# titisda/graph-python

Hardware: AMD Instinct MI355X
Metric: GTEPS (masked mxv/vxm level-BFS, R-MAT s22) (higher is better)
Workload: dtype bool; 1 GPU; level-BFS q<!v.S,replace> = q any.pair A (GxB_ANY_PAIR_BOOL; GrB_vxm, GrB_mxv on A^T shards for N>1), R-MAT scale 22, edge factor 16, 16 roots; n=4194304, nnz=65243197, parallelism=single GPU

## Files before the change

### graph-python_amd/csrc/gb_internal.h

```cpp
#pragma once
#include <atomic>
#include <utility>
#include <hip/hip_runtime.h>

#include <cstdint>
#include <cstring>
#include <stdexcept>
#include <string>
#include <vector>

#include "../../include/gbamd_codes.h"
#include "gb_state.h"
#include "../../include/graphblas_amd.h"

#define GB_MAGIC 0x6d614d424731ULL
#define GB_FREED 0x646565724642ULL

struct GB_Type_opaque {
    uint64_t magic;
    int code;
    size_t size;
    const char *name;
};
struct GB_BinaryOp_opaque {
// ... 1 lines not shown
    int opcode;
    GrB_Type xtype, ytype, ztype;
    const char *name;
};
struct GB_UnaryOp_opaque {
    uint64_t magic;
    int opcode;
    GrB_Type xtype, ztype;
    const char *name;
};
struct GB_IndexUnaryOp_opaque {
    uint64_t magic;
    int opcode;
    GrB_Type xtype, ytype;
    const char *name;
};
struct GB_Monoid_opaque {
    uint64_t magic;
    int mcode;
    GrB_Type type;
    GrB_BinaryOp op;
    const char *name;
};
struct GB_Semiring_opaque {
    uint64_t magic;
    GrB_Monoid add;
    GrB_BinaryOp mul;
    const char *name;
    bool user;
};
struct GB_Descriptor_opaque {
    uint64_t magic;
    int outp, mask, inp0, inp1;
    bool builtin;
    const char *name;
};

struct GB_builtin_entry {
    const char *name;
    int kind;
    void *obj;
};
extern const GB_builtin_entry GB_builtin_registry[];

enum { GB_KIND_MATRIX = 0, GB_KIND_VECTOR = 1, GB_KIND_SCALAR = 2 };

struct gb_orient_cache {
    int32_t *hub_tab = nullptr;
    int64_t hub_n = 0, hub_H = 0;
    uint64_t *rows_ne = nullptr;
    uint32_t *ne_rank = nullptr;
    int32_t *phead = nullptr;
    uint32_t *pdeg = nullptr;
    int64_t maxdeg = -1;
    int32_t *long_tab = nullptr;
    int64_t long_n = 0;
    int32_t *hot_ci = nullptr;
    int32_t *hot_cols = nullptr;
    int64_t hot_n = 0;
    void *nar_vx = nullptr;
    int nar_k = 0;
    bool nar_done = false;
};
void gb_orient_cache_drop(gb_orient_cache &c);

struct GB_Matrix_opaque {
    uint64_t magic;
    int kind;
    GrB_Type type;
    int64_t nrows, ncols;
    bool iso;
    int64_t nvals;
    int64_t *rowptr;
    int32_t *colidx;
    void *vals;
    bool t_valid;
    int64_t *t_rowptr;
    int32_t *t_colidx;
    void *t_vals;
    int64_t *t_perm;
    gb_orient_cache oc[2];
    uint64_t *bits;
    void *dense;
    int64_t *d_nvals;
    bool nvals_valid;
    struct gb_host_slot *pub;
    uint64_t pub_seq, pub_epoch;
    bool hint_valid;
    const void *hint_key;
    std::string err;
    uint64_t *cw;
    void *cw_vals;
    int64_t *cw_stat;
    GrB_Info invalid = GrB_SUCCESS;
};
typedef GB_Matrix_opaque GB_Obj;

inline GB_Obj *OBJ(const void *p) { return (GB_Obj *)p; }

struct gb_exception {
    GrB_Info info;
    std::string msg;
};
[[noreturn]] void gb_throw(GrB_Info info, const std::string &msg);
#define GB_REQUIRE(cond, info, msg) \
    do {                            \
// ... 104 lines not shown
void *gb_malloc(size_t bytes);
void gb_free(void *p);
template <class T>
T *gb_malloc_n(size_t n) {
    return (T *)gb_malloc(n * sizeof(T));
}
void gb_memset(void *p, int v, size_t bytes);
void gb_copy_d2d(void *dst, const void *src, size_t bytes);
void gb_copy_h2d(void *dst, const void *src, size_t bytes);
void gb_copy_d2h(void *dst, const void *src, size_t bytes);

struct gb_scratch {
    void *ptrs[32];
    int n = 0;
    template <class T>
    T *get(size_t count) {
        T *p = gb_malloc_n<T>(count ? count : 1);
        ptrs[n++] = p;
        return p;
    }
    ~gb_scratch() {
        for (int i = 0; i < n; i++) gb_free(ptrs[i]);
    }
};

GB_Obj *gb_obj_check(const void *p, bool allow_null = false);
GB_Obj *gb_obj_check_raw(const void *p, bool allow_null = false);
void gb_cw_to_csr(GB_Obj *A);
void gb_cw_release(GB_Obj *A);
void gb_cw_materialize(GB_Obj *A);
GB_Obj *gb_new_object(int kind, GrB_Type type, int64_t nrows, int64_t ncols);
extern "C" void gb_vec_recount(GB_Obj *v);
void gb_obj_free_storage(GB_Obj *A);
void gb_drop_transpose(GB_Obj *A);
int64_t gb_nvals(GB_Obj *A);
inline int64_t gb_words(int64_t n) { return (n + 63) >> 6; }
inline bool gb_is_bitmap(const GB_Obj *A) { return A->kind != GB_KIND_MATRIX; }

void gb_cast_array(void *dst, int dst_code, const void *src, int src_code, int64_t n);

struct gb_csr_view {
    int64_t nrows = 0, ncols = 0, nvals = 0;
    const int64_t *rowptr = nullptr;
    const int32_t *colidx = nullptr;
    const void *vals = nullptr;
    bool iso = false;
    int tcode = 0;
    const int32_t *hubs = nullptr;
    int64_t nhubs = 0, hub_H = 0;
    const uint64_t *nonempty = nullptr;
    const uint32_t *ne_rank = nullptr;
    const int32_t *phead = nullptr;
    const uint32_t *pdeg = nullptr;
    int64_t maxdeg = -1;
    const int32_t *lchunks = nullptr;
    int64_t nlchunks = -1;
    const void *nvx = nullptr;
    int nvk = 0;
    const int32_t *hcolidx = nullptr;
    const int32_t *hcols = nullptr;
    int64_t nhot = 0;
    gb_scratch own;
};
void gb_get_csr(gb_csr_view &v, GB_Obj *A);
void gb_view_hubs(gb_csr_view &v, GB_Obj *A, int orient, int64_t H);
void gb_view_nonempty(gb_csr_view &v, GB_Obj *A, int orient);
void gb_view_pullfirst(gb_csr_view &v, GB_Obj *A, int orient, const int64_t *other_rowptr, int64_t other_n);
void gb_view_long_rows(gb_csr_view &v, GB_Obj *A, int orient);
void gb_view_narrow(gb_csr_view &v, GB_Obj *A, int orient);
void gb_view_hot(gb_csr_view &v, GB_Obj *A, int orient);
void gb_get_csc(gb_csr_view &v, GB_Obj *A);
const int64_t *gb_csc_perm(GB_Obj *A);
const void *gb_view_vals_as(gb_csr_view &v, int code, gb_scratch &s);

struct gb_bitmap_view {
    int64_t n = 0;
    const uint64_t *bits = nullptr;
    const void *vals = nullptr;
    bool iso = false;
    int tcode = 0;
    const int64_t *count = nullptr;
    const long long *mf_hint = nullptr;
    const void *hint_key = nullptr;
    bool full = false;
    int64_t h_nvals = -1;
    gb_scratch own;
};
void gb_get_bitmap(gb_bitmap_view &v, GB_Obj *A);
const void *gb_bitmap_vals_as(gb_bitmap_view &v, int code, gb_scratch &s);

void gb_install_csr(GB_Obj *C, int64_t nrows, int64_t ncols, int64_t nvals, int64_t *rowptr,
                    int32_t *colidx, void *vals, bool iso);
void gb_install_bitmap(GB_Obj *C, int64_t n, uint64_t *bits, void *dense, bool iso,
                       int64_t *d_nvals );

void gb_bitmap_count(const uint64_t *bits, int64_t n, int64_t *d_count);
void gb_bitmap_to_csr(const uint64_t *bits, const void *dense, bool iso, int64_t n, size_t tsize,
                      int64_t **rowptr, int32_t **colidx, void **vals, int64_t *nvals);
void gb_csr_col_to_bitmap(const gb_csr_view &v, size_t tsize, uint64_t **bits, void **dense,
                          int64_t **d_nvals);

void gb_build(GB_Obj *C, const GrB_Index *I, const GrB_Index *J, const void *X, int xcode, bool x_iso,
              int64_t n, GrB_BinaryOp dup);
void gb_extract_tuples(GB_Obj *A, GrB_Index *I, GrB_Index *J, void *X, int xcode, GrB_Index *nvals);

void *gb_expand_iso(const void *one_value, size_t tsize, int64_t n);
// ... 163 lines not shown
```

### graph-python_amd/csrc/gb_mxv.hip

```cpp
#include "gb_dispatch.cuh"
#include "gb_internal.h"

#define SPMV_TILE 256

template <class SR, class X, class Z, bool FLIP>
__global__ __launch_bounds__(SPMV_BLOCK) void k_spmv_pull(
    SR sr, int64_t nrows, const int64_t *__restrict__ rowptr, const int32_t *__restrict__ colidx,
    const X *__restrict__ avals, bool a_iso, const uint64_t *__restrict__ ubits,
    const X *__restrict__ uvals, bool u_iso, const uint64_t *__restrict__ mbits, bool mcomp, int lg,
    uint64_t *__restrict__ tbits, Z *__restrict__ tvals, unsigned long long *__restrict__ tcount,
    unsigned long long *__restrict__ gst) {
    __shared__ unsigned long long words[SPMV_TILE / 64];
    const int G = 1 << lg;
    const int gid = threadIdx.x >> lg;
    const int gl = threadIdx.x & (G - 1);
    const int ngroups = SPMV_BLOCK >> lg;
    const int lane = threadIdx.x & 63;
    const unsigned long long gmask = (G == 64) ? ~0ULL : (((1ULL << G) - 1) << (lane & ~(G - 1)));
    const int64_t nwords = (nrows + 63) >> 6;
    const bool rv = SR::reads_values && avals && uvals;
    X a0 = X(), u0 = X();
    if (rv) {
        if (a_iso) a0 = avals[0];
        if (u_iso) u0 = uvals[0];
// ... 511 lines not shown
    const int64_t nw = (n + 63) >> 6;
    for (int64_t w = (blockIdx.x * (int64_t)blockDim.x + threadIdx.x) >> 6; w < nw;
         w += ((int64_t)gridDim.x * blockDim.x) >> 6) {
        const int64_t r = (w << 6) + lane;
        const unsigned long long b = __ballot(r < n && rowptr[r + 1] > rowptr[r]);
        if (lane == 0) {
            ne[w] = b;
            pc[w] = __popcll(b);
        }
    }
}

__global__ void k_narrow_u32(const int64_t *__restrict__ in, uint32_t *__restrict__ out, int64_t n) {
    GB_GRID_LOOP(i, n)
        out[i] = (uint32_t)in[i];
}

void gb_view_nonempty(gb_csr_view &v, GB_Obj *A, int orient) {
    if (A->kind != GB_KIND_MATRIX) return;
    gb_orient_cache &c = A->oc[orient];
    if (!c.rows_ne) {
        const int64_t nw = gb_words(v.nrows);
        c.rows_ne = gb_malloc_n<uint64_t>(nw);
        c.ne_rank = gb_malloc_n<uint32_t>(nw + 1);
        if (nw == 0) {
            gb_memset(c.ne_rank, 0, sizeof(uint32_t));
        } else {
            gb_scratch s;
            int32_t *pc = s.get<int32_t>(nw);
            int64_t *pre = s.get<int64_t>(nw + 1);
            const unsigned g = (unsigned)std::max<int64_t>(1, std::min<int64_t>((nw + 3) / 4, 8192));
            hipLaunchKernelGGL(k_rows_nonempty, dim3(g), dim3(256), 0, gb_stream(), v.rowptr, v.nrows, c.rows_ne, pc);
            GB_LAUNCH_CHECK();
            gb_exclusive_scan_i32(pc, 0, pre, nw);
            hipLaunchKernelGGL(k_narrow_u32, dim3(gb_grid(nw + 1, 256, 4096)), dim3(256), 0, gb_stream(), pre,
                               c.ne_rank, nw + 1);
            GB_LAUNCH_CHECK();
        }
    }
    v.nonempty = c.rows_ne;
    v.ne_rank = c.ne_rank;
}

__device__ __forceinline__ void pf_better(int64_t &bd, int32_t &bi, int64_t d, int32_t i) {
    if (i >= 0 && (d > bd || (d == bd && (bi < 0 || i < bi)))) {
        bd = d;
        bi = i;
    }
}
__global__ __launch_bounds__(256) void k_pull_head(int64_t n, const int64_t *__restrict__ rp,
                                                   const int32_t *__restrict__ ci,
                                                   const int64_t *__restrict__ orp, int64_t on,
                                                   const uint64_t *__restrict__ ne, const uint32_t *__restrict__ rank,
                                                   int4 *__restrict__ head, uint32_t *__restrict__ pdeg) {
    const int lane = threadIdx.x & 63;
    const int64_t nwaves = ((int64_t)gridDim.x * blockDim.x) >> 6;
    for (int64_t j = (blockIdx.x * (int64_t)blockDim.x + threadIdx.x) >> 6; j < n; j += nwaves) {
        const int64_t e0 = rp[j], e1 = rp[j + 1], d = e1 - e0;
        if (d <= 0) continue;
        const int64_t slot = (int64_t)rank[j >> 6] + __popcll(ne[j >> 6] & ((1ULL << (j & 63)) - 1));
        int32_t pick[4] = {-1, -1, -1, -1};
        const int rounds = d <= 4 ? (int)d : 3;
        for (int r = 0; r < rounds; r++) {
            int64_t bd = -1;
            int32_t bi = -1;
            for (int64_t e = e0 + lane; e < e1; e += 64) {
                const int32_t i = ci[e];
                bool taken = false;
                for (int q = 0; q < r; q++) taken = taken || pick[q] == i;
                if (!taken) pf_better(bd, bi, orp[i + 1] - orp[i], i);
            }
            for (int off = 32; off > 0; off >>= 1) {
                const int64_t od = __shfl_xor(bd, off, 64);
                const int32_t oi = __shfl_xor(bi, off, 64);
                pf_better(bd, bi, od, oi);
            }
            pick[r] = bi;
        }
        if (d > 4) pick[3] = -2;
        if (lane == 0) {
            head[slot] = make_int4(pick[0], pick[1], pick[2], pick[3]);
            if (pdeg) {
                const int64_t od = j < on ? orp[j + 1] - orp[j] : 0;
                pdeg[slot] = (uint32_t)(od < 0xFFFFFFFFLL ? od : 0xFFFFFFFFLL);
            }
        }
    }
}

void gb_view_pullfirst(gb_csr_view &v, GB_Obj *A, int orient, const int64_t *other_rowptr, int64_t other_n) {
    if (A->kind != GB_KIND_MATRIX || v.nrows == 0) return;
    gb_orient_cache &c = A->oc[orient];
    if (!c.rows_ne || !c.ne_rank || v.nonempty != c.rows_ne || v.ne_rank != c.ne_rank) return;
    if (!c.phead) {
        uint32_t ne_count = 0;
        gb_copy_d2h(&ne_count, c.ne_rank + gb_words(v.nrows), sizeof(ne_count));
        const int64_t nrec = std::max<int64_t>(1, (int64_t)ne_count);
        c.phead = gb_malloc_n<int32_t>(4 * nrec);
        c.pdeg = gb_malloc_n<uint32_t>(nrec);
        const unsigned g = (unsigned)std::max<int64_t>(1, std::min<int64_t>((v.nrows + 3) / 4, 65535));
        hipLaunchKernelGGL(k_pull_head, dim3(g), dim3(256), 0, gb_stream(), v.nrows, v.rowptr, v.colidx,
                           other_rowptr, other_n, c.rows_ne, c.ne_rank, reinterpret_cast<int4 *>(c.phead), c.pdeg);
        GB_LAUNCH_CHECK();
    }
    v.phead = c.phead;
    v.pdeg = c.pdeg;
}

static bool idempotent_monoid(int m) {
    return m == GBAMD_MON_ANY || m == GBAMD_MON_MIN || m == GBAMD_MON_MAX || m == GBAMD_MON_LOR ||
           m == GBAMD_MON_LAND || m == GBAMD_MON_BOR || m == GBAMD_MON_BAND;
}

bool gb_spmv_result_iso(GrB_Semiring sr, bool a_iso, bool u_iso, bool flip) {
    gb_sr_info info = gb_sr_describe(sr);
    bool reads_a = info.reads_values, reads_u = info.reads_values;
    if (info.mul == GBAMD_OP_FIRST) (flip ? reads_a : reads_u) = false;
    if (info.mul == GBAMD_OP_SECOND) (flip ? reads_u : reads_a) = false;
    if (info.mul == GBAMD_OP_PAIR) return idempotent_monoid(info.mon);
    return !info.positional && idempotent_monoid(info.mon) && (!reads_a || a_iso) && (!reads_u || u_iso);
}

template <class F>
static void gb_with_flip(bool flip, F &&f) {
    if (flip) f(std::true_type{});
    else f(std::false_type{});
}

void gb_spmv(gb_vec_result &T, const gb_csr_view &A, const gb_csr_view *Apush, gb_bitmap_view &u,
             const gb_vmask &mask, GrB_Semiring sr, bool flip, const gb_asg *asg) {
    gb_sr_info info = gb_sr_describe(sr);
    gb_scratch s;
    gb_csr_view &Av = const_cast<gb_csr_view &>(A);
    const void *av = info.reads_values ? gb_view_vals_as(Av, info.xcode, s) : nullptr;
    const void *uv = info.reads_values ? gb_bitmap_vals_as(u, info.xcode, s) : nullptr;
    const bool iso = gb_spmv_result_iso(sr, A.iso, u.iso, flip);

    const int64_t n = A.nrows;
    const size_t zs = gb_type_size(info.zcode);
    T.n = n;
    T.tcode = info.zcode;
    T.iso = iso;
    T.bits = gb_malloc_n<uint64_t>(gb_words(n));
    T.dense = gb_malloc((iso ? 1 : n) * zs);
    T.d_nvals = gb_malloc_n<int64_t>(2 + GB_HINT_PARTS);
    if (n == 0) {
        gb_memset(T.d_nvals, 0, sizeof(int64_t));
        return;
    }

    if (iso) {
        gb_spmv_iso(T, A, Apush, u, mask, sr, flip, asg, av, uv);
        return;
    }
    const int64_t nw = gb_words(n);
    unsigned long long *gst = gb_device_state();

    gb_dispatch_sr(info, [&](auto srf, auto x, auto z) {
        using SRT = decltype(srf);
// ... 54 lines not shown
```

### graph-python_amd/csrc/gb_object.hip

```cpp
#include <algorithm>
#include <vector>

#include <mutex>

#include "gb_dispatch.cuh"
#include "gb_internal.h"

#define GB_BLOCK 256
#define OBJ_GRID_CAP 8192

GB_Obj *gb_obj_check(const void *p, bool allow_null) {
    GB_Obj *A = gb_obj_check_raw(p, allow_null);
    if (A && A->cw) gb_cw_to_csr(A);
    return A;
}

GB_Obj *gb_obj_check_raw(const void *p, bool allow_null) {
    if (!p) {
        if (allow_null) return nullptr;
        gb_throw(GrB_NULL_POINTER, "required object is NULL");
    }
    GB_Obj *A = OBJ(p);
    if (A->magic == GB_FREED) gb_throw(GrB_INVALID_OBJECT, "object has been freed");
    if (A->magic != GB_MAGIC) gb_throw(GrB_UNINITIALIZED_OBJECT, "object is not initialized");
// ... 27 lines not shown
    GB_REQUIRE(type && type->magic == GB_MAGIC, GrB_UNINITIALIZED_OBJECT, "invalid type");
    GB_REQUIRE(nrows >= 0 && ncols >= 0, GrB_INVALID_VALUE, "negative dimension");
    GB_REQUIRE(nrows <= (int64_t)GrB_INDEX_MAX && ncols <= (int64_t)GrB_INDEX_MAX, GrB_INVALID_VALUE,
               "dimension too large");
    if (kind == GB_KIND_MATRIX) {
        GB_REQUIRE(ncols < (1LL << 31), GrB_OUT_OF_MEMORY,
                   "matrix with >= 2^31 columns exceeds the device index width");
    }
    GB_Obj *A = new GB_Obj();
    A->magic = GB_MAGIC;
    A->kind = kind;
    A->type = type;
    A->nrows = nrows;
    A->ncols = ncols;
    return A;
}

GB_Obj *gb_new_object(int kind, GrB_Type type, int64_t nrows, int64_t ncols) {
    GB_Obj *A = gb_new_object_bare(kind, type, nrows, ncols);
    try {
        alloc_empty_storage(A);
    } catch (...) {
        gb_free(A->rowptr);
        gb_free(A->bits);
        gb_free(A->d_nvals);
        A->magic = GB_FREED;
        delete A;
        throw;
    }
    return A;
}

void gb_drop_transpose(GB_Obj *A) {
    if (A->t_valid) {
        gb_free(A->t_rowptr);
        gb_free(A->t_colidx);
        gb_free(A->t_vals);
        gb_free(A->t_perm);
    }
    A->t_perm = nullptr;
    A->t_rowptr = nullptr;
    A->t_colidx = nullptr;
    A->t_vals = nullptr;
    A->t_valid = false;
    for (gb_orient_cache &c : A->oc) gb_orient_cache_drop(c);
}

void gb_orient_cache_drop(gb_orient_cache &c) {
    gb_free(c.hub_tab);
    gb_free(c.rows_ne);
    gb_free(c.ne_rank);
    gb_free(c.phead);
    gb_free(c.pdeg);
    gb_free(c.long_tab);
    gb_free(c.hot_ci);
    gb_free(c.hot_cols);
    gb_free(c.nar_vx);
    c = gb_orient_cache{};
}

void gb_obj_free_storage(GB_Obj *A) {
    gb_cw_release(A);
    gb_drop_transpose(A);
    gb_free(A->rowptr);
    gb_free(A->colidx);
    gb_free(A->vals);
    gb_free(A->bits);
    gb_free(A->dense);
    A->rowptr = nullptr;
    A->colidx = nullptr;
    A->vals = nullptr;
    A->bits = nullptr;
    A->dense = nullptr;
}

std::atomic<int64_t> g_stat_nvals_copy{0};
std::atomic<int64_t> g_stat_host_push{0};

int64_t gb_nvals(GB_Obj *A) {
    if (A->kind == GB_KIND_MATRIX && !A->cw) return A->nvals;
    if (!A->nvals_valid) {
        int64_t v;
        if (A->pub && A->pub_seq && A->pub_epoch == gb_epoch() && gb_host_slot_wait(A->pub, A->pub_seq, &v)) {
            A->nvals = v;
        } else {
            g_stat_nvals_copy.fetch_add(1, std::memory_order_relaxed);
            A->nvals = gb_read_i64(A->cw ? A->cw_stat : A->d_nvals);
        }
        A->nvals_valid = true;
    }
    return A->nvals;
}

void gb_install_csr(GB_Obj *C, int64_t nrows, int64_t ncols, int64_t nvals, int64_t *rowptr,
                    int32_t *colidx, void *vals, bool iso) {
    if (C->kind == GB_KIND_MATRIX) {
        gb_cw_release(C);
        gb_drop_transpose(C);
        gb_free(C->rowptr);
        gb_free(C->colidx);
        gb_free(C->vals);
        C->nrows = nrows;
        C->ncols = ncols;
        C->nvals = nvals;
        C->rowptr = rowptr;
        C->colidx = colidx;
// ... 1333 lines not shown
```

### graph-python_amd/csrc/gb_spmv_iso.hip

```cpp
#include <mutex>

#include "gb_dispatch.cuh"
#include "gb_internal.h"

enum { ST_PUSH = 0 };
#define PULL_U 4

struct gb_dir_rule {
    const int64_t *mask_count;
    const int64_t *extra_count;
    bool mcomp;
    int64_t n_out, nnz, alpha;
    int force_push;
};

__device__ __forceinline__ bool gb_dir_decide(long long mf, const gb_dir_rule &rule) {
    int64_t open = rule.n_out;
    if (rule.mask_count) {
        int64_t mc = *rule.mask_count;
        if (rule.extra_count) mc += *rule.extra_count;
        if (mc > rule.n_out) mc = rule.n_out;
        open = rule.mcomp ? (rule.n_out - mc) : mc;
    }
    const double avg = rule.n_out ? (double)rule.nnz / (double)rule.n_out : 0.0;
// ... 522 lines not shown
            }
#pragma unroll
            for (int u = 0; u < PULL_U; u++) {
                if (go[u]) {
                    int f = 0;
                    if (dbg & 32) {
#pragma unroll
                        for (int t = 0; t < 4; t++) f += k[u][t] == 0x7fffffff;
                    } else {
#pragma unroll
                        for (int t = 0; t < 4; t++) f += k[u][t] >= 0 && gb_bit(ubits, k[u][t]);
                    }
                    found[u] = f != 0;
                    p[u] += 4;
                }
            }
        }
        int n = 0;
#pragma unroll
        for (int u = 0; u < PULL_U; u++) {
            const bool pd = live[u] && !found[u] && p[u] < p1[u];
            const unsigned long long bb = __ballot(pd);
            if (pd) {
                const int i = n + __popcll(bb & lt);
                L.p[i] = p[u];
                L.rem[i] = (int32_t)(p1[u] - p[u]);
                L.id[i] = (int16_t)(u * 64 + lane);
            }
            n += __popcll(bb);
        }
        if (lane < PULL_U) L.hitw[lane] = 0;
        if (dbg & 16) n = 0;
        gb_wlist_walk_pull(L, n, cap0, colidx, ubits);
#pragma unroll
        for (int u = 0; u < PULL_U; u++) {
            if ((L.hitw[u] >> lane) & 1ULL) found[u] = true;
            const unsigned long long word = __ballot(found[u]);
            if (lane == 0 && w0 + u < nwords) {
                tbits[w0 + u] = word;
                cnt += __popcll(word);
            }
        }
        if (hprow) {
#pragma unroll
            for (int u = 0; u < PULL_U; u++)
                if (found[u]) mfn += dg[u];
        }
    }
    return cnt;
}

#define PACK_G 4
#define PACK_W (PACK_G * PULL_U)
struct gb_wpack {
    int16_t ids[PACK_W * 64];
    unsigned long long fw[PACK_W];
    unsigned long long rw[PACK_W];
    uint32_t rk[PACK_W];
};
__device__ __forceinline__ long long gb_pull_iso_packed(int64_t nrows, const int64_t *__restrict__ rowptr,
                                                       const int32_t *__restrict__ colidx,
                                                       const uint64_t *__restrict__ ubits,
                                                       const uint64_t *__restrict__ mbits, bool mcomp,
                                                       uint64_t *__restrict__ tbits, gb_wlist &L, gb_wpack &P,
                                                       const int64_t *__restrict__ hprow, long long &mfn, int cap0,
                                                       const uint64_t *__restrict__ rne,
                                                       const uint64_t *__restrict__ qbits, const gb_asg_dev &g,
                                                       long long &adelta, const int32_t *__restrict__ ph,
                                                       const uint32_t *__restrict__ pdeg,
                                                       const uint32_t *__restrict__ nrk) {
    const int lane = threadIdx.x & 63;
    const int64_t wave = (blockIdx.x * (int64_t)blockDim.x + threadIdx.x) >> 6;
    const int64_t nwaves = ((int64_t)gridDim.x * blockDim.x) >> 6;
    const int64_t nwords = (nrows + 63) >> 6;
    const int64_t stride = nwaves * PULL_U;
    const uint64_t tail = (nrows & 63) ? ((1ULL << (nrows & 63)) - 1) : ~0ULL;
    const unsigned long long lt = (1ULL << lane) - 1;
    long long cnt = 0;
    for (int64_t wb = wave * PULL_U; wb < nwords; wb += stride * PACK_G) {
        const int64_t wl = wb + (int64_t)(lane / PULL_U) * stride + (lane & (PULL_U - 1));
        const bool inr = lane < PACK_W && wl < nwords;
        const uint64_t qw = (qbits && inr) ? qbits[wl] : 0;
        const uint64_t mw = (mbits && inr) ? mbits[wl] : 0;
        const uint64_t rw = (rne && inr) ? rne[wl] : ~0ULL;
        const uint32_t nr = inr ? nrk[wl] : 0;
        uint64_t mine = ~0ULL;
        if (qbits) {
            if (qw) {
                const uint64_t c = g.bits == mbits ? mw : g.bits[wl], nwd = c | qw;
                if (nwd != c) g.bits[wl] = nwd;
                adelta += (long long)__popcll(nwd) - (long long)__popcll(c);
            }
            for (unsigned long long qb = __ballot(qw != 0); qb; qb &= qb - 1) {
                const int u = __ffsll(qb) - 1;
                const uint64_t word = __shfl(qw, u, 64);
                const int64_t wu = wb + (int64_t)(u / PULL_U) * stride + (u & (PULL_U - 1));
                if ((word >> lane) & 1ULL) gb_store_sized(g.vals, (wu << 6) + lane, g.size, g.x);
            }
            if (mbits) mine = mcomp ? ~(mw | qw) : (mw | qw);
        } else if (mbits) {
            mine = mcomp ? ~mw : mw;
        }
        if (rne) mine &= rw;
        if (wl == nwords - 1) mine &= tail;
        if (!inr) mine = 0;
        const int c = __popcll(mine);
        int incl = c;
#pragma unroll
        for (int off = 1; off < PACK_W; off <<= 1) {
            const int y = __shfl_up(incl, off, 64);
            if (lane >= off) incl += y;
        }
        const int excl = incl - c;
        const int total = __shfl(incl, PACK_W - 1, 64);
        if (!total) {
            if (inr) tbits[wl] = 0;
            continue;
        }
        const unsigned long long ob = __ballot(mine != 0);
        for (unsigned long long b = ob; b; b &= b - 1) {
            const int u = __ffsll(b) - 1;
            const uint64_t word = __shfl(mine, u, 64);
            const int base = __shfl(excl, u, 64);
            if ((word >> lane) & 1ULL) P.ids[base + __popcll(word & lt)] = (int16_t)(u * 64 + lane);
        }
        if (lane < PACK_W) {
            P.rw[lane] = rw;
            P.rk[lane] = nr;
        }
        gb_wave_sync();
        for (int b0 = 0; b0 < total; b0 += 256) {
            bool live[PULL_U], found[PULL_U];
            int64_t r[PULL_U];
            uint32_t rk[PULL_U];
            int4 hv[PULL_U];
#pragma unroll
            for (int u = 0; u < PULL_U; u++) {
                const int i = b0 + u * 64 + lane;
                live[u] = i < total;
                const int id = live[u] ? P.ids[i] : 0;
                r[u] = ((wb + (int64_t)(id >> 8) * stride + ((id >> 6) & (PULL_U - 1))) << 6) + (id & 63);
                rk[u] = gb_ne_rank(P.rk[id >> 6], P.rw[id >> 6], id & 63);
                hv[u] = make_int4(-1, -1, -1, -1);
                if (live[u]) hv[u] = reinterpret_cast<const int4 *>(ph)[rk[u]];
            }
            gb_pull_probe_heads(hv, ubits, found);
            int64_t p[PULL_U], p1[PULL_U], dg[PULL_U];
#pragma unroll
            for (int u = 0; u < PULL_U; u++) {
                p[u] = p1[u] = 0;
                if (live[u] && !found[u] && hv[u].w == -2 && r[u] < nrows) {
                    p[u] = rowptr[r[u]];
                    p1[u] = rowptr[r[u] + 1];
                }
                dg[u] = (hprow && found[u]) ? (int64_t)pdeg[rk[u]] : p1[u] - p[u];
            }
            int n = 0;
#pragma unroll
            for (int u = 0; u < PULL_U; u++) {
                const bool pd = p[u] < p1[u];
                const unsigned long long bb = __ballot(pd);
                if (pd) {
                    const int i = n + __popcll(bb & lt);
                    L.p[i] = p[u];
                    L.rem[i] = (int32_t)(p1[u] - p[u]);
                    L.id[i] = (int16_t)(u * 64 + lane);
                }
                n += __popcll(bb);
            }
            if (lane < PULL_U) L.hitw[lane] = 0;
            gb_wlist_walk_pull(L, n, cap0, colidx, ubits);
#pragma unroll
            for (int u = 0; u < PULL_U; u++) {
                if ((L.hitw[u] >> lane) & 1ULL) found[u] = true;
                const unsigned long long word = __ballot(found[u]);
                if (lane == 0) P.fw[(b0 >> 6) + u] = word;
                if (hprow && found[u]) mfn += dg[u];
            }
            gb_wave_sync();
        }
        unsigned long long res = 0;
        for (unsigned long long b = ob; b; b &= b - 1) {
            const int u = __ffsll(b) - 1;
            const uint64_t word = __shfl(mine, u, 64);
            const int base = __shfl(excl, u, 64);
            bool f = false;
            if ((word >> lane) & 1ULL) {
                const int i = base + __popcll(word & lt);
                f = (P.fw[i >> 6] >> (i & 63)) & 1ULL;
            }
            const unsigned long long fb = __ballot(f);
            if (lane == u) res = fb;
        }
        if (inr) {
            tbits[wl] = res;
            cnt += __popcll(res);
        }
        gb_wave_sync();
    }
    return cnt;
}

template <class X>
__device__ void gb_iso_eval_x(int mul, bool zbool, bool flip, const void *a0, const void *u0, void *out) {
    const X a = a0 ? *(const X *)a0 : X(), b = u0 ? *(const X *)u0 : X();
    const X x = flip ? b : a, y = flip ? a : b;
    if (zbool) *(bool *)out = gb_binop_z<X, bool>(mul, x, y, 0, 0, 0);
    else *(X *)out = gb_binop_z<X, X>(mul, x, y, 0, 0, 0);
}
__device__ void gb_iso_eval(int mul, int xcode, int zcode, bool flip, const void *a0, const void *u0, void *out) {
    const bool zb = zcode == GBAMD_T_BOOL && xcode != GBAMD_T_BOOL;
    switch (xcode) {
    case GBAMD_T_BOOL: gb_iso_eval_x<bool>(mul, zb, flip, a0, u0, out); break;
    case GBAMD_T_INT8: gb_iso_eval_x<int8_t>(mul, zb, flip, a0, u0, out); break;
    case GBAMD_T_UINT8: gb_iso_eval_x<uint8_t>(mul, zb, flip, a0, u0, out); break;
    case GBAMD_T_INT16: gb_iso_eval_x<int16_t>(mul, zb, flip, a0, u0, out); break;
    case GBAMD_T_UINT16: gb_iso_eval_x<uint16_t>(mul, zb, flip, a0, u0, out); break;
    case GBAMD_T_INT32: gb_iso_eval_x<int32_t>(mul, zb, flip, a0, u0, out); break;
    case GBAMD_T_UINT32: gb_iso_eval_x<uint32_t>(mul, zb, flip, a0, u0, out); break;
    case GBAMD_T_INT64: gb_iso_eval_x<int64_t>(mul, zb, flip, a0, u0, out); break;
    case GBAMD_T_UINT64: gb_iso_eval_x<uint64_t>(mul, zb, flip, a0, u0, out); break;
    case GBAMD_T_FP32: gb_iso_eval_x<float>(mul, zb, flip, a0, u0, out); break;
    case GBAMD_T_FP64: gb_iso_eval_x<double>(mul, zb, flip, a0, u0, out); break;
    default: break;
    }
}

#define GB_ZP_MAX 4

struct gb_iso_args {
    const long long *mf_hint;
    gb_dir_rule rule;
    const unsigned long long *dst;
    const int64_t *hprow;
    long long *mf_out;
    int mul, xcode, zcode;
    bool flip;
    const void *a0, *u0;
    void *iso_out;
    gb_host_slot *pub;
    long long pub_seq;
    int pub_form;
    const int64_t *u_exit;
    bool out_zeroed;
    uint64_t *spare;
    int64_t spare_words;
    int p1_steps, cap0;
    int dbg;
    int pack;
    bool packed;
    const uint64_t *rows_nonempty;
    const uint32_t *ne_rank;
    const int32_t *phead;
    const uint32_t *pdeg;
    int host_dir;
    uint64_t *zb[GB_ZP_MAX];
    int64_t *zc[GB_ZP_MAX];
    int nzb, nzc;
    int64_t zb_words;
    gb_asg_dev asg;
    const void *asg_qiso;
    int asg_qiso_code;
    unsigned long long *asg_count;
    int64_t root;
    unsigned long long *ts;
};

#define ISO_ARR_BITS 10
#define ISO_VAL_BITS 27

#define ISO_TS_PAIRS (1 << 20)
__device__ __forceinline__ void iso_ts_mark(const gb_iso_args &a, int which) {
    if (!a.ts) return;
    const unsigned long long t = __builtin_amdgcn_s_memrealtime();
    const unsigned long long k = atomicAdd(&a.ts[which], 1ULL);
    if (k < ISO_TS_PAIRS) a.ts[2 + 2 * k + which] = t;
}

__device__ __forceinline__ void iso_publish(const gb_iso_args &a, long long tot) {
    iso_ts_mark(a, 1);
    if (!a.pub || (a.dbg & 1)) return;
    if (a.pub_form == 1) {
        __hip_atomic_store(&a.pub->value, tot, __ATOMIC_RELAXED, __HIP_MEMORY_SCOPE_SYSTEM);
        __threadfence_system();
        __hip_atomic_store(&a.pub->seq, a.pub_seq, __ATOMIC_RELEASE, __HIP_MEMORY_SCOPE_SYSTEM);
        return;
    }
    const long long w = (long long)(GB_PUB_TAG | (((unsigned long long)a.pub_seq & 0x7fffffffULL) << 32) |
                                    ((unsigned long long)tot & 0xffffffffULL));
    if (a.pub_form == 0) __hip_atomic_store(&a.pub->seq, w, __ATOMIC_RELAXED, __HIP_MEMORY_SCOPE_SYSTEM);
    else __hip_atomic_store(&a.pub->seq, w, __ATOMIC_RELEASE, __HIP_MEMORY_SCOPE_SYSTEM);
}
__device__ __forceinline__ void iso_finish_packed(long long cnt, long long mfn, long long adelta,
                                                  unsigned long long *__restrict__ tcount,
                                                  unsigned long long *__restrict__ gst, const gb_iso_args &a) {
    __shared__ long long part[3][SPMV_BLOCK / 64];
    for (int off = 32; off > 0; off >>= 1) {
        cnt += __shfl_xor(cnt, off, 64);
        mfn += __shfl_xor(mfn, off, 64);
        adelta += __shfl_xor(adelta, off, 64);
    }
    const int wid = threadIdx.x >> 6;
    if ((threadIdx.x & 63) == 0) {
        part[0][wid] = cnt;
        part[1][wid] = mfn;
        part[2][wid] = adelta;
    }
// ... 3 lines not shown
    for (int w = 0; w < SPMV_BLOCK / 64; w++) {
        cnt += part[0][w];
        mfn += part[1][w];
        adelta += part[2][w];
    }
    const unsigned nb = gridDim.x;
    const unsigned s = blockIdx.x % GB_GRID_SHARDS;
    const unsigned in_shard = (nb - s + GB_GRID_SHARDS - 1) / GB_GRID_SHARDS;
    const unsigned long long AM = (1ULL << ISO_ARR_BITS) - 1, VM = (1ULL << ISO_VAL_BITS) - 1;
    unsigned long long *cs = gst + (size_t)s * GB_GRID_STRIDE;
    unsigned long long *hs = gst + GB_GRID2_OFFSET + (size_t)s * GB_GRID_STRIDE;
    const unsigned long long pk =
        ((unsigned long long)adelta << (ISO_ARR_BITS + ISO_VAL_BITS)) | ((unsigned long long)cnt << ISO_ARR_BITS) | 1ULL;
    unsigned long long oh = 0;
    if (a.mf_out) {
        oh = atomicAdd(hs, ((unsigned long long)mfn << 12) + 1ULL);
        if (blockIdx.x == 0)
            for (unsigned i = nb; i < GB_HINT_PARTS; i++) a.mf_out[i] = 0;
    }
    const unsigned long long oc = atomicAdd(cs, pk);
    if (a.mf_out && (unsigned)(oh & 0xFFF) + 1 == in_shard) {
        a.mf_out[s] = (long long)(oh >> 12) + mfn;
        atomicExch(hs, 0ULL);
    }
    if ((unsigned)(oc & AM) + 1 != in_shard) return;
    atomicExch(cs, 0ULL);
    const unsigned long long scnt = ((oc >> ISO_ARR_BITS) & VM) + (unsigned long long)cnt;
    const unsigned long long sadd = (oc >> (ISO_ARR_BITS + ISO_VAL_BITS)) + (unsigned long long)adelta;
    const unsigned nshards = nb < GB_GRID_SHARDS ? nb : GB_GRID_SHARDS;
    unsigned long long *root = gst + (size_t)GB_GRID_SHARDS * GB_GRID_STRIDE;
    const unsigned long long o2 =
        atomicAdd(root, (sadd << (ISO_ARR_BITS + ISO_VAL_BITS)) | (scnt << ISO_ARR_BITS) | 1ULL);
    if ((unsigned)(o2 & AM) + 1 != nshards) return;
    const long long tot = (long long)(((o2 >> ISO_ARR_BITS) & VM) + scnt);
    const long long add = (long long)((o2 >> (ISO_ARR_BITS + ISO_VAL_BITS)) + sadd);
    *tcount = (unsigned long long)tot;
    iso_publish(a, tot);
    atomicExch(root, 0ULL);
    if (a.asg.bits && add) atomicAdd(a.asg_count, (unsigned long long)add);
}

__global__ __launch_bounds__(SPMV_BLOCK) void k_iso_work(
    int64_t nrows, const int64_t *__restrict__ rowptr, const int32_t *__restrict__ colidx,
    int64_t nwords_u, const uint64_t *__restrict__ ubits, const int64_t *__restrict__ prow,
    const int32_t *__restrict__ pcol, const int32_t *__restrict__ hubs, int64_t nhubs, int64_t H,
    const uint64_t *__restrict__ mbits, bool mcomp, uint64_t *__restrict__ tbits,
    unsigned long long *__restrict__ tcount, unsigned long long *__restrict__ gst, gb_iso_args a) {
    __shared__ gb_wlist lists[WAVES_PER_BLOCK];
    gb_wlist &L = lists[threadIdx.x >> 6];
    __shared__ gb_wpack packs[WAVES_PER_BLOCK];
    if (a.ts && blockIdx.x == 0 && threadIdx.x == 0) iso_ts_mark(a, 0);
    if (a.dbg & 8) return;
    bool push = false;
    if (a.host_dir == 1) {
        push = true;
    } else if (a.mf_hint) {
        long long mf = 0;
        for (int i = 0; i < GB_HINT_PARTS; i++) mf += a.mf_hint[i];
        push = gb_dir_decide(mf, a.rule);
    }
    else if (a.dst) push = a.dst[ST_PUSH] != 0;
    if (a.spare && !(a.dbg & 32)) {
        for (int64_t w = blockIdx.x * (int64_t)blockDim.x + threadIdx.x; w < a.spare_words;
             w += (int64_t)gridDim.x * blockDim.x)
            a.spare[w] = 0;
    }
    for (int j = 0; j < ((a.dbg & 32) ? 0 : a.nzb); j++)
        for (int64_t w = blockIdx.x * (int64_t)blockDim.x + threadIdx.x; w < a.zb_words;
             w += (int64_t)gridDim.x * blockDim.x)
            a.zb[j][w] = 0;
    if (blockIdx.x == 0)
        for (int j = 0; j < a.nzc; j++)
            for (int w = threadIdx.x; w < 2 + GB_HINT_PARTS; w += blockDim.x) a.zc[j][w] = 0;
    if (a.packed && a.iso_out && blockIdx.x == 0 && threadIdx.x == 0)
        gb_iso_eval(a.mul, a.xcode, a.zcode, a.flip, a.a0, a.u0, a.iso_out);
    if (a.u_exit && *a.u_exit == 0) {
        if (!a.out_zeroed)
            for (int64_t w = blockIdx.x * (int64_t)blockDim.x + threadIdx.x; w < ((nrows + 63) >> 6);
                 w += (int64_t)gridDim.x * blockDim.x)
                tbits[w] = 0;
        if (blockIdx.x == 0) {
            if (a.mf_out)
                for (int i = threadIdx.x; i < GB_HINT_PARTS; i += blockDim.x) a.mf_out[i] = 0;
            if (threadIdx.x == 0) {
                *tcount = 0ULL;
                if (!a.packed && a.iso_out) gb_iso_eval(a.mul, a.xcode, a.zcode, a.flip, a.a0, a.u0, a.iso_out);
                iso_publish(a, 0);
            }
        }
        return;
    }
    const uint64_t *qbits = nullptr;
    if (a.asg.bits && (!a.asg_qiso || gb_dyn_nonzero(a.asg_qiso, a.asg_qiso_code))) qbits = ubits;
    long long mfn = 0, cnt = 0, adelta = 0;
    if (a.dbg & 4)
        ;
    else if (a.root >= 0)
        cnt = gb_push_root(a.root, prow, pcol, mbits, mcomp, (unsigned long long *)tbits, a.hprow, mfn,
                           a.asg.bits != nullptr, a.asg, adelta);
    else if (push)
        cnt = gb_push_phase(nwords_u, ubits, prow, pcol, hubs, nhubs, H, mbits, mcomp,
                            (unsigned long long *)tbits, L, a.hprow, mfn, qbits, a.asg, adelta, (a.dbg & 128) != 0,
                            (a.dbg & 512) == 0, (a.pack & 2) != 0);
    else {
        const int32_t *ph =
            (a.phead && a.rows_nonempty && a.ne_rank && (!a.hprow || a.pdeg)) ? a.phead : nullptr;
        if ((a.pack & 1) && ph && a.p1_steps == 0 && !(a.dbg & (16 | 32 | 128)))
            cnt = gb_pull_iso_packed(nrows, rowptr, colidx, ubits, mbits, mcomp, tbits, L, packs[threadIdx.x >> 6],
                                     a.hprow, mfn, a.cap0, a.rows_nonempty, qbits, a.asg, adelta, ph, a.pdeg, a.ne_rank);
        else
            cnt = gb_pull_iso_phase(nrows, rowptr, colidx, ubits, mbits, mcomp, tbits, L, a.hprow, mfn, a.p1_steps,
                                    a.cap0, a.rows_nonempty, qbits, a.asg, adelta, a.dbg, ph, a.pdeg, a.ne_rank);
    }
    if (a.dbg & 64) return;
    if (a.packed) {
        iso_finish_packed(cnt, mfn, adelta, tcount, gst, a);
        return;
    }
    long long tot;
    if (gb_grid_sum(cnt, gst, &tot)) {
        *tcount = (unsigned long long)tot;
        if (a.iso_out) gb_iso_eval(a.mul, a.xcode, a.zcode, a.flip, a.a0, a.u0, a.iso_out);
        iso_publish(a, tot);
    }
    if (a.mf_out && !(a.dbg & 2)) {
        long long m;
        if (gb_grid_sum(mfn, gst + GB_GRID2_OFFSET, &m)) {
            a.mf_out[0] = m;
            for (int i = 1; i < GB_HINT_PARTS; i++) a.mf_out[i] = 0;
        }
    }
    if (a.asg.bits) gb_grid_add(adelta, a.asg_count, gst + GB_GRID3_OFFSET);
}

static std::mutex g_dir_mu;
static unsigned long long *g_iso_ts = nullptr;
static unsigned long long *iso_ts_buffer() {
    static const bool on = getenv("GRAPHBLAS_AMD_ISO_TS") != nullptr;
    if (!on) return nullptr;
    if (!g_iso_ts) {
        GB_HIP(hipMalloc((void **)&g_iso_ts, (2 + 2 * (size_t)ISO_TS_PAIRS) * sizeof(unsigned long long)));
        GB_HIP(hipMemset(g_iso_ts, 0, (2 + 2 * (size_t)ISO_TS_PAIRS) * sizeof(unsigned long long)));
        GB_HIP(hipDeviceSynchronize());
    }
    return g_iso_ts;
}
int64_t gb_iso_ts_dump() {
    const char *path = getenv("GRAPHBLAS_AMD_ISO_TS");
    if (!path || !g_iso_ts) return 0;
    GB_HIP(hipStreamSynchronize(gb_stream()));
    unsigned long long c[2];
    GB_HIP(hipMemcpy(c, g_iso_ts, sizeof(c), hipMemcpyDeviceToHost));
    const size_t k = std::min<unsigned long long>(std::min(c[0], c[1]), ISO_TS_PAIRS);
    std::vector<unsigned long long> buf(2 + 2 * k);
    GB_HIP(hipMemcpy(buf.data(), g_iso_ts, buf.size() * sizeof(unsigned long long), hipMemcpyDeviceToHost));
    FILE *f = fopen(path, "wb");
    if (!f) return -1;
    fwrite(buf.data(), sizeof(unsigned long long), buf.size(), f);
    fclose(f);
    return (int64_t)k;
}
static uint64_t *g_spare = nullptr;
// ... 40 lines not shown
    static int64_t cap = 0;
    if (!cap) {
        int dev = 0, cus = 0, per = 0;
        GB_HIP(hipGetDevice(&dev));
        GB_HIP(hipDeviceGetAttribute(&cus, hipDeviceAttributeMultiprocessorCount, dev));
        GB_HIP(hipOccupancyMaxActiveBlocksPerMultiprocessor(&per, k_iso_work, SPMV_BLOCK, 0));
        cap = std::max<int64_t>(1, (int64_t)cus * std::max(per, 1));
    }
    return cap;
}

void gb_spmv_iso(gb_vec_result &T, const gb_csr_view &A, const gb_csr_view *Apush, gb_bitmap_view &u,
                 const gb_vmask &mask, GrB_Semiring sr, bool flip, const gb_asg *asg, const void *av,
                 const void *uv) {
    const gb_sr_info info = gb_sr_describe(sr);
    GB_REQUIRE(info.zcode == info.xcode || info.zcode == GBAMD_T_BOOL, GrB_NOT_IMPLEMENTED,
               "semiring type combination not supported");
    const int64_t n = A.nrows;
    const int64_t dir_knob = gb_knob("spmv_direction");
    const bool can_push = Apush && Apush->nrows == u.n && Apush->hubs && dir_knob != 1;
    int64_t alpha = gb_knob("push_alpha");
    if (alpha <= 0) alpha = 48;
    const int64_t nw = gb_words(n);
    unsigned long long *gst = gb_device_state();
    unsigned long long *dst = gst + GB_DIR_STATE_OFFSET;
    const int64_t uw = gb_words(u.n);
    int64_t units = (nw + PULL_U - 1) / PULL_U;
    std::lock_guard<std::mutex> lk(g_dir_mu);
    gb_iso_args args{};
    args.rule = gb_dir_rule{mask.count, asg ? u.count : nullptr, mask.comp, n, A.nvals, alpha, dir_knob == 2};
    if (asg) {
        GB_REQUIRE(u.n == n, GrB_INVALID_VALUE, "fused assign needs u and w of one size");
        args.asg = gb_asg_dev{asg->bits, asg->vals, asg->size, asg->x};
        args.asg_qiso = asg->q_iso;
        args.asg_qiso_code = asg->q_iso_code;
        args.asg_count = (unsigned long long *)asg->count;
    }
    args.dbg = (int)gb_knob("iso_dbg");
    const int64_t pack_knob = gb_knob("iso_pack");
    args.pack = ((pack_knob == 0 || pack_knob == 2) ? 1 : 0) | ((pack_knob == 0 || pack_knob == 3) ? 2 : 0);
    args.ts = iso_ts_buffer();
    args.root = asg ? asg->root : -1;
    GB_REQUIRE(args.root < 0 || can_push, GrB_PANIC, "a pending root needs the push orientation");
    args.packed = n < (1LL << ISO_VAL_BITS) && u.n < (1LL << ISO_VAL_BITS) && gb_knob("iso_packed") != 1;
    if (args.dbg & 1) T.pub = nullptr;
    args.p1_steps = (int)gb_knob("pull_steps");
    if (args.p1_steps < 0) args.p1_steps = 0;
    args.cap0 = (int)gb_knob("pull_cap");
    if (args.cap0 <= 0) args.cap0 = 64;
    args.rows_nonempty = A.nonempty;
    args.ne_rank = A.ne_rank;
    args.phead = A.phead;
    args.pdeg = A.pdeg;
    args.mul = info.mul;
    args.xcode = info.xcode;
    args.zcode = info.zcode;
    args.flip = flip;
    args.a0 = av;
    args.u0 = uv;
    args.iso_out = T.dense;
    args.pub = T.pub ? gb_host_slot_device(T.pub) : nullptr;
    args.pub_seq = (long long)T.pub_seq;
    args.pub_form = n < (1LL << 31) ? (int)std::max<int64_t>(0, std::min<int64_t>(2, gb_knob("iso_pub"))) : 1;
    bool spare_taken = false;
    if (g_spare && g_spare_words == nw) {
        gb_free(T.bits);
        T.bits = g_spare;
        spare_taken = true;
    } else if (g_spare) {
        gb_free(g_spare);
    }
    g_spare = nullptr;
    g_spare_words = 0;
    args.out_zeroed = spare_taken;
    if (asg && asg->u_count_exact && u.count && asg->root < 0 && gb_knob("spec_empty_exit") != 1)
        args.u_exit = u.count;
    bool need_prep = false;
    if (can_push) {
        units = std::max<int64_t>(units, std::max<int64_t>((Apush->nhubs + 15) / 16, (uw + 3) / 4));
        if (n == u.n) {
            args.hprow = Apush->rowptr;
            args.mf_out = (long long *)(T.d_nvals + 2);
            T.hint_key = Apush->rowptr;
        }
        const bool hint_ok = u.mf_hint && u.hint_key == Apush->rowptr;
        bool push_sure = false;
        if (!hint_ok && spare_taken && u.h_nvals >= 0 && Apush->maxdeg >= 0 &&
            gb_knob("host_dir") != 1) {
            int64_t open_lo = -1;
            if (!mask.bits) {
                open_lo = n;
            } else if (mask.h_count >= 0) {
                const int64_t mc_hi = std::min<int64_t>(n, mask.h_count + (asg ? u.h_nvals : 0));
                open_lo = mask.comp ? n - mc_hi : mask.h_count;
            }
            const double avg = n ? (double)A.nvals / (double)n : 0.0;
            push_sure = open_lo >= 0 &&
                        (double)u.h_nvals * (double)Apush->maxdeg * (double)alpha < (double)open_lo * avg;
        }
        if (args.root >= 0) {
            if (!spare_taken) gb_memset(T.bits, 0, nw * sizeof(uint64_t));
            args.out_zeroed = true;
            args.host_dir = 1;
            g_stat_host_push.fetch_add(1, std::memory_order_relaxed);
            gb_stat_add("bfs_root_push", 1);
        } else if (hint_ok && spare_taken) {
// ... 62 lines not shown
```

Measured before the change: 350.0 GTEPS.

## Add compact first-parent table and wide first-probe pass in packed pull BFS

Builds a new per-nonempty-row int2 table holding the best candidate parent and saturated degree, then in the packed pull kernel first probes that single parent for 8 wavefronts-worth of rows at once. Only rows that miss go on to the full head probe and adjacency walk, and their found bits are merged back with shared atomics. The aim is to cut the 16-byte head loads and to keep more probes in flight when most rows find a parent on the first candidate. The cost is extra memory for the table, a second level of compaction with LDS atomics, and a heuristic that enables the wide pass only in heavy pull levels.

```diff
diff --git a/graph-python_amd/csrc/gb_internal.h b/graph-python_amd/csrc/gb_internal.h
--- a/graph-python_amd/csrc/gb_internal.h
+++ b/graph-python_amd/csrc/gb_internal.h
@@ -77,6 +77,7 @@
     uint32_t *ne_rank = nullptr;
     int32_t *phead = nullptr;
     uint32_t *pdeg = nullptr;
+    int32_t *pfirst = nullptr;
     int64_t maxdeg = -1;
     int32_t *long_tab = nullptr;
     int64_t long_n = 0;
@@ -287,6 +288,7 @@
     const uint32_t *ne_rank = nullptr;
     const int32_t *phead = nullptr;
     const uint32_t *pdeg = nullptr;
+    const int32_t *pfirst = nullptr;
     int64_t maxdeg = -1;
     const int32_t *lchunks = nullptr;
     int64_t nlchunks = -1;
diff --git a/graph-python_amd/csrc/gb_mxv.hip b/graph-python_amd/csrc/gb_mxv.hip
--- a/graph-python_amd/csrc/gb_mxv.hip
+++ b/graph-python_amd/csrc/gb_mxv.hip
@@ -587,7 +587,8 @@
                                                    const int32_t *__restrict__ ci,
                                                    const int64_t *__restrict__ orp, int64_t on,
                                                    const uint64_t *__restrict__ ne, const uint32_t *__restrict__ rank,
-                                                   int4 *__restrict__ head, uint32_t *__restrict__ pdeg) {
+                                                   int4 *__restrict__ head, uint32_t *__restrict__ pdeg,
+                                                   int2 *__restrict__ first) {
     const int lane = threadIdx.x & 63;
     const int64_t nwaves = ((int64_t)gridDim.x * blockDim.x) >> 6;
     for (int64_t j = (blockIdx.x * (int64_t)blockDim.x + threadIdx.x) >> 6; j < n; j += nwaves) {
@@ -617,7 +618,9 @@
             head[slot] = make_int4(pick[0], pick[1], pick[2], pick[3]);
             if (pdeg) {
                 const int64_t od = j < on ? orp[j + 1] - orp[j] : 0;
-                pdeg[slot] = (uint32_t)(od < 0xFFFFFFFFLL ? od : 0xFFFFFFFFLL);
+                const uint32_t sat = (uint32_t)(od < 0xFFFFFFFFLL ? od : 0xFFFFFFFFLL);
+                pdeg[slot] = sat;
+                if (first) first[slot] = make_int2(pick[0], (int)sat);
             }
         }
     }
@@ -633,13 +636,16 @@
         const int64_t nrec = std::max<int64_t>(1, (int64_t)ne_count);
         c.phead = gb_malloc_n<int32_t>(4 * nrec);
         c.pdeg = gb_malloc_n<uint32_t>(nrec);
+        c.pfirst = gb_malloc_n<int32_t>(2 * nrec);
         const unsigned g = (unsigned)std::max<int64_t>(1, std::min<int64_t>((v.nrows + 3) / 4, 65535));
         hipLaunchKernelGGL(k_pull_head, dim3(g), dim3(256), 0, gb_stream(), v.nrows, v.rowptr, v.colidx,
-                           other_rowptr, other_n, c.rows_ne, c.ne_rank, reinterpret_cast<int4 *>(c.phead), c.pdeg);
+                           other_rowptr, other_n, c.rows_ne, c.ne_rank, reinterpret_cast<int4 *>(c.phead), c.pdeg,
+                           reinterpret_cast<int2 *>(c.pfirst));
         GB_LAUNCH_CHECK();
     }
     v.phead = c.phead;
     v.pdeg = c.pdeg;
+    v.pfirst = c.pfirst;
 }
 
 static bool idempotent_monoid(int m) {
diff --git a/graph-python_amd/csrc/gb_object.hip b/graph-python_amd/csrc/gb_object.hip
--- a/graph-python_amd/csrc/gb_object.hip
+++ b/graph-python_amd/csrc/gb_object.hip
@@ -103,6 +103,7 @@
     gb_free(c.ne_rank);
     gb_free(c.phead);
     gb_free(c.pdeg);
+    gb_free(c.pfirst);
     gb_free(c.long_tab);
     gb_free(c.hot_ci);
     gb_free(c.hot_cols);
diff --git a/graph-python_amd/csrc/gb_spmv_iso.hip b/graph-python_amd/csrc/gb_spmv_iso.hip
--- a/graph-python_amd/csrc/gb_spmv_iso.hip
+++ b/graph-python_amd/csrc/gb_spmv_iso.hip
@@ -598,12 +598,16 @@
 
 #define PACK_G 4
 #define PACK_W (PACK_G * PULL_U)
+#define PACK_WIDE 8
+#define PULL_WIDE_SHARE 6
 struct gb_wpack {
     int16_t ids[PACK_W * 64];
     unsigned long long fw[PACK_W];
     unsigned long long rw[PACK_W];
     uint32_t rk[PACK_W];
+    int16_t miss[PACK_WIDE * 64];
 };
+
 __device__ __forceinline__ long long gb_pull_iso_packed(int64_t nrows, const int64_t *__restrict__ rowptr,
                                                        const int32_t *__restrict__ colidx,
                                                        const uint64_t *__restrict__ ubits,
@@ -614,7 +618,8 @@
                                                        const uint64_t *__restrict__ qbits, const gb_asg_dev &g,
                                                        long long &adelta, const int32_t *__restrict__ ph,
                                                        const uint32_t *__restrict__ pdeg,
-                                                       const uint32_t *__restrict__ nrk) {
+                                                       const uint32_t *__restrict__ nrk,
+                                                       const int32_t *__restrict__ pf) {
     const int lane = threadIdx.x & 63;
     const int64_t wave = (blockIdx.x * (int64_t)blockDim.x + threadIdx.x) >> 6;
     const int64_t nwaves = ((int64_t)gridDim.x * blockDim.x) >> 6;
@@ -675,55 +680,98 @@
             P.rk[lane] = nr;
         }
         gb_wave_sync();
-        for (int b0 = 0; b0 < total; b0 += 256) {
-            bool live[PULL_U], found[PULL_U];
-            int64_t r[PULL_U];
-            uint32_t rk[PULL_U];
-            int4 hv[PULL_U];
-#pragma unroll
-            for (int u = 0; u < PULL_U; u++) {
-                const int i = b0 + u * 64 + lane;
-                live[u] = i < total;
-                const int id = live[u] ? P.ids[i] : 0;
-                r[u] = ((wb + (int64_t)(id >> 8) * stride + ((id >> 6) & (PULL_U - 1))) << 6) + (id & 63);
-                rk[u] = gb_ne_rank(P.rk[id >> 6], P.rw[id >> 6], id & 63);
-                hv[u] = make_int4(-1, -1, -1, -1);
-                if (live[u]) hv[u] = reinterpret_cast<const int4 *>(ph)[rk[u]];
-            }
-            gb_pull_probe_heads(hv, ubits, found);
-            int64_t p[PULL_U], p1[PULL_U], dg[PULL_U];
-#pragma unroll
-            for (int u = 0; u < PULL_U; u++) {
-                p[u] = p1[u] = 0;
-                if (live[u] && !found[u] && hv[u].w == -2 && r[u] < nrows) {
-                    p[u] = rowptr[r[u]];
-                    p1[u] = rowptr[r[u] + 1];
-                }
-                dg[u] = (hprow && found[u]) ? (int64_t)pdeg[rk[u]] : p1[u] - p[u];
-            }
-            int n = 0;
-#pragma unroll
-            for (int u = 0; u < PULL_U; u++) {
-                const bool pd = p[u] < p1[u];
-                const unsigned long long bb = __ballot(pd);
-                if (pd) {
-                    const int i = n + __popcll(bb & lt);
-                    L.p[i] = p[u];
-                    L.rem[i] = (int32_t)(p1[u] - p[u]);
-                    L.id[i] = (int16_t)(u * 64 + lane);
-                }
-                n += __popcll(bb);
-            }
-            if (lane < PULL_U) L.hitw[lane] = 0;
-            gb_wlist_walk_pull(L, n, cap0, colidx, ubits);
-#pragma unroll
-            for (int u = 0; u < PULL_U; u++) {
-                if ((L.hitw[u] >> lane) & 1ULL) found[u] = true;
-                const unsigned long long word = __ballot(found[u]);
-                if (lane == 0) P.fw[(b0 >> 6) + u] = word;
-                if (hprow && found[u]) mfn += dg[u];
-            }
-            gb_wave_sync();
+        const uint32_t *ub32 = reinterpret_cast<const uint32_t *>(ubits);
+        for (int b0 = 0; b0 < total; b0 += pf ? PACK_WIDE * 64 : PULL_U * 64) {
+            int nm = total - b0 < PULL_U * 64 ? total - b0 : PULL_U * 64;
+            if (pf) {
+                bool live[PACK_WIDE];
+                int2 fh[PACK_WIDE];
+#pragma unroll
+                for (int u = 0; u < PACK_WIDE; u++) {
+                    const int i = b0 + u * 64 + lane;
+                    live[u] = i < total;
+                    const int id = live[u] ? P.ids[i] : 0;
+                    fh[u] = make_int2(-1, 0);
+                    if (live[u])
+                        fh[u] = reinterpret_cast<const int2 *>(pf)[gb_ne_rank(P.rk[id >> 6], P.rw[id >> 6], id & 63)];
+                }
+                uint32_t w1[PACK_WIDE];
+#pragma unroll
+                for (int u = 0; u < PACK_WIDE; u++) {
+                    w1[u] = 0;
+                    if (fh[u].x >= 0) w1[u] = ub32[fh[u].x >> 5];
+                }
+                nm = 0;
+#pragma unroll
+                for (int u = 0; u < PACK_WIDE; u++) {
+                    const bool f = fh[u].x >= 0 && ((w1[u] >> (fh[u].x & 31)) & 1u);
+                    if (hprow && f) mfn += (long long)(uint32_t)fh[u].y;
+                    const unsigned long long fb = __ballot(f);
+                    if (lane == 0) P.fw[(b0 >> 6) + u] = fb;
+                    const bool ms = live[u] && !f;
+                    const unsigned long long mb = __ballot(ms);
+                    if (ms) P.miss[nm + __popcll(mb & lt)] = (int16_t)(u * 64 + lane);
+                    nm += __popcll(mb);
+                }
+                gb_wave_sync();
+            }
+            for (int s0 = 0; s0 < nm; s0 += PULL_U * 64) {
+                bool found[PULL_U];
+                int slot[PULL_U];
+                int64_t r[PULL_U];
+                uint32_t rk[PULL_U];
+                int4 hv[PULL_U];
+#pragma unroll
+                for (int u = 0; u < PULL_U; u++) {
+                    const int j = s0 + u * 64 + lane;
+                    const bool lv = j < nm;
+                    slot[u] = !lv ? 0 : pf ? (int)P.miss[j] : j;
+                    const int id = lv ? P.ids[b0 + slot[u]] : 0;
+                    r[u] = ((wb + (int64_t)(id >> 8) * stride + ((id >> 6) & (PULL_U - 1))) << 6) + (id & 63);
+                    rk[u] = gb_ne_rank(P.rk[id >> 6], P.rw[id >> 6], id & 63);
+                    hv[u] = make_int4(-1, -1, -1, -1);
+                    if (lv) hv[u] = reinterpret_cast<const int4 *>(ph)[rk[u]];
+                    if (pf) hv[u].x = -1;
+                }
+                gb_pull_probe_heads(hv, ubits, found);
+                int64_t p[PULL_U], p1[PULL_U], dg[PULL_U];
+#pragma unroll
+                for (int u = 0; u < PULL_U; u++) {
+                    p[u] = p1[u] = 0;
+                    if (!found[u] && hv[u].w == -2 && r[u] < nrows) {
+                        p[u] = rowptr[r[u]];
+                        p1[u] = rowptr[r[u] + 1];
+                    }
+                    dg[u] = (hprow && found[u]) ? (int64_t)pdeg[rk[u]] : p1[u] - p[u];
+                }
+                int n = 0;
+#pragma unroll
+                for (int u = 0; u < PULL_U; u++) {
+                    const bool pd = p[u] < p1[u];
+                    const unsigned long long bb = __ballot(pd);
+                    if (pd) {
+                        const int i = n + __popcll(bb & lt);
+                        L.p[i] = p[u];
+                        L.rem[i] = (int32_t)(p1[u] - p[u]);
+                        L.id[i] = (int16_t)(u * 64 + lane);
+                    }
+                    n += __popcll(bb);
+                }
+                if (lane < PULL_U) L.hitw[lane] = 0;
+                gb_wlist_walk_pull(L, n, cap0, colidx, ubits);
+#pragma unroll
+                for (int u = 0; u < PULL_U; u++) {
+                    if ((L.hitw[u] >> lane) & 1ULL) found[u] = true;
+                    if (pf) {
+                        if (found[u]) atomicOr(&P.fw[(b0 >> 6) + (slot[u] >> 6)], 1ULL << (slot[u] & 63));
+                    } else {
+                        const unsigned long long word = __ballot(found[u]);
+                        if (lane == 0) P.fw[(b0 >> 6) + u] = word;
+                    }
+                    if (hprow && found[u]) mfn += dg[u];
+                }
+                gb_wave_sync();
+            }
         }
         unsigned long long res = 0;
         for (unsigned long long b = ob; b; b &= b - 1) {
@@ -799,6 +847,8 @@
     const uint32_t *ne_rank;
     const int32_t *phead;
     const uint32_t *pdeg;
+    const int32_t *pfirst;
+    bool wide_all;
     int host_dir;
     uint64_t *zb[GB_ZP_MAX];
     int64_t *zc[GB_ZP_MAX];
@@ -908,12 +958,14 @@
     if (a.ts && blockIdx.x == 0 && threadIdx.x == 0) iso_ts_mark(a, 0);
     if (a.dbg & 8) return;
     bool push = false;
+    long long mf_in = -1;
     if (a.host_dir == 1) {
         push = true;
     } else if (a.mf_hint) {
         long long mf = 0;
         for (int i = 0; i < GB_HINT_PARTS; i++) mf += a.mf_hint[i];
         push = gb_dir_decide(mf, a.rule);
+        mf_in = mf;
     }
     else if (a.dst) push = a.dst[ST_PUSH] != 0;
     if (a.spare && !(a.dbg & 32)) {
@@ -961,9 +1013,11 @@
     else {
         const int32_t *ph =
             (a.phead && a.rows_nonempty && a.ne_rank && (!a.hprow || a.pdeg)) ? a.phead : nullptr;
+        const bool wide = a.wide_all || mf_in < 0 || mf_in * PULL_WIDE_SHARE > a.rule.nnz;
         if ((a.pack & 1) && ph && a.p1_steps == 0 && !(a.dbg & (16 | 32 | 128)))
             cnt = gb_pull_iso_packed(nrows, rowptr, colidx, ubits, mbits, mcomp, tbits, L, packs[threadIdx.x >> 6],
-                                     a.hprow, mfn, a.cap0, a.rows_nonempty, qbits, a.asg, adelta, ph, a.pdeg, a.ne_rank);
+                                     a.hprow, mfn, a.cap0, a.rows_nonempty, qbits, a.asg, adelta, ph, a.pdeg, a.ne_rank,
+                                     wide ? a.pfirst : nullptr);
         else
             cnt = gb_pull_iso_phase(nrows, rowptr, colidx, ubits, mbits, mcomp, tbits, L, a.hprow, mfn, a.p1_steps,
                                     a.cap0, a.rows_nonempty, qbits, a.asg, adelta, a.dbg, ph, a.pdeg, a.ne_rank);
@@ -1110,6 +1164,9 @@
     args.ne_rank = A.ne_rank;
     args.phead = A.phead;
     args.pdeg = A.pdeg;
+    const int64_t wide_knob = gb_knob("pull_wide");
+    args.pfirst = wide_knob == 1 ? nullptr : A.pfirst;
+    args.wide_all = wide_knob == 2;
     args.mul = info.mul;
     args.xcode = info.xcode;
     args.zcode = info.zcode;
```

After: 352.3 GTEPS, median of 6. About the same (+0.6%).
